# AndrewCullacino/handwritten-chinese-ocr-samples

Hardware: AMD Instinct MI355X
Metric: text-lines/sec (1x128x2000 synth) greedy decode (higher is better)
Workload: dtype f16 (f32 accumulate); 1 GPU; BASELINE configs[1]: 64 x 1x128x2000 uint8 lines, random-init hctr checkpoint (C=7358), forward + greedy CTC decode, labels to host; global_lines=64, lines_per_gpu=64, width=2000, classes=7358, checkpoint=random, parallelism=batch-shard x1

## Files before the change

handwritten-chinese-ocr-samples_amd/csrc/engine.cpp:

```cpp
#include "../../include/hctr_hip.h"
#include "kernels.h"

#include <algorithm>
#include <cfloat>
#include <cmath>
#include <cstdarg>
#include <cstdio>
#include <cstring>
#include <map>
#include <new>
#include <string>
#include <vector>

using namespace hctr;

namespace {

constexpr int kImgH = 128;
constexpr int kFeat = 2048;
constexpr double kBnEps = 1e-5;
constexpr int kStagePlanes[4] = {128, 256, 512, 512};
constexpr int kStageBlocks[4] = {2, 4, 5, 1};
constexpr int kStageH[5] = {128, 64, 32, 16, 8};
constexpr int64_t kDefaultMaxCols = 131072;

std::string g_create_error;

struct HostTensor {
    std::vector<float> data;
    std::vector<int64_t> shape;
    mutable bool used = false;
};

struct ConvW {
    half_t* w = nullptr;
    float* bias = nullptr;
    int cin = 0, cout = 0, coutPad = 0, taps = 0;
};

struct SeW {
    float* w1 = nullptr;
    float* w2 = nullptr;
    int c = 0;
};

struct BlockW {
    ConvW conv1, conv2, ds;
    SeW se;
    bool has_ds = false;
};

struct Workspace {
    int B = 0, W = 0, Wa = 0;
    void* img = nullptr;
    int32_t* widths = nullptr;
    half_t* s0 = nullptr;
    half_t* x[5] = {};
    half_t* p[5][3] = {};
    half_t* headin = nullptr;
    float* logits = nullptr;
    float* se_part = nullptr;
    float* se_scale = nullptr;
    float* se_border = nullptr;
    float* se_mean = nullptr;
    int32_t* se_counter = nullptr;
    int32_t* colidx = nullptr;
    float* amax_val = nullptr;
    int32_t* amax_idx = nullptr;
    int32_t* labels = nullptr;
    int32_t* lengths = nullptr;
    float* psum = nullptr;
    float* blank_logit = nullptr;
    float* row_thr = nullptr;
    int32_t* emit_cnt = nullptr;
    int32_t* emit_list = nullptr;
    double* esum = nullptr;
    int32_t* overflow = nullptr;
    int32_t* bm_idx = nullptr;
    float* bm_lp = nullptr;
    float* bm_bl = nullptr;
    float* bm_st = nullptr;
    int32_t* bm_cnt = nullptr;
    int32_t* tile_ctrs = nullptr;
    float* amax_val2 = nullptr;
    float* amax_abs = nullptr;
    float* col_margin = nullptr;
    float* col_abs = nullptr;
    float* line_guard = nullptr;
    int features = 0;
    bool split = false;
    bool aliased = false;
};

enum WsFeature { WS_S0 = 1, WS_LOGITS = 2, WS_BEAM = 4, WS_GUARD = 8 };

struct WeightSet {
    float* stem_w = nullptr;
    float* stem_b = nullptr;
    ConvW conv0_2;
    std::vector<BlockW> blocks[4];
    ConvW stage_conv[4];
    ConvW head;
    bool built = false;
};

struct ProfEntry {
    std::string name;
    hipEvent_t e0, e1;
};

}

struct hctr_ctx {
    int device = 0;
    int num_classes = 0;
    int cpad = 0;
    hipStream_t stream = nullptr;
    std::string err;
    std::map<std::string, HostTensor> host;
// ... 112 lines not shown
    for (void* p : pool) (void)hipFree(p);
    pool.clear();
}

struct PoolGuard {
    std::vector<void*>& pool;
    ~PoolGuard() { free_pool(pool); }
};

const HostTensor* find(hctr_ctx* c, const std::string& key) {
    auto it = c->host.find(key);
    return it == c->host.end() ? nullptr : &it->second;
}

int need(hctr_ctx* c, const std::string& key, std::vector<int64_t> shape, const HostTensor** out) {
    const HostTensor* t = find(c, key);
    if (!t) return fail(c, HCTR_ERR_KEY, "Missing key(s) in state_dict: \"%s\"", key.c_str());
    if (t->shape != shape) {
        std::string got, want;
        for (auto v : t->shape) got += std::to_string(v) + ",";
        for (auto v : shape) want += std::to_string(v) + ",";
        return fail(c, HCTR_ERR_SHAPE, "size mismatch for %s: checkpoint [%s] vs model [%s]", key.c_str(),
                    got.c_str(), want.c_str());
    }
    t->used = true;
    *out = t;
    return HCTR_OK;
}

inline int perm64(int s) {
    const int j = s >> 4, ra = s & 15;
    return (j >> 1) * 32 + (ra >> 2) * 8 + (j & 1) * 4 + (ra & 3);
}

int build_conv(hctr_ctx* c, const std::string& ck, const std::string& bk, int cin, int cout, int ks,
               bool has_bias, int pad_to, ConvW* out) {
    const HostTensor *w, *b = nullptr, *g, *beta, *mean, *var;
    TRY(need(c, ck + ".weight", {cout, cin, ks, ks}, &w));
    if (has_bias) TRY(need(c, ck + ".bias", {cout}, &b));
    TRY(need(c, bk + ".weight", {cout}, &g));
    TRY(need(c, bk + ".bias", {cout}, &beta));
    TRY(need(c, bk + ".running_mean", {cout}, &mean));
    TRY(need(c, bk + ".running_var", {cout}, &var));
    const int taps = ks * ks;
    const int coutPad = (cout + pad_to - 1) / pad_to * pad_to;
    const int cinp = c->chm() * cin;
    std::vector<half_t> hw((size_t)taps * coutPad * cinp, (half_t)0.f);
    std::vector<float> hb(coutPad, 0.f);
    double wmax = 0.0;
    for (int blk = 0; blk < coutPad / 64; ++blk)
        for (int s = 0; s < 64; ++s) {
            const int co = blk * 64 + perm64(s);
            if (co >= cout) continue;
            const double sc = (double)g->data[co] / std::sqrt((double)var->data[co] + kBnEps);
            for (int t = 0; t < taps; ++t)
                for (int ci = 0; ci < cin; ++ci) {
                    const double v = (double)w->data[((size_t)co * cin + ci) * taps + t] * sc;
                    wmax = std::max(wmax, std::fabs(v));
                    half_t* row = &hw[((size_t)t * coutPad + blk * 64 + s) * cinp];
                    const half_t hi = (half_t)(float)v;
                    row[ci] = hi;
                    if (c->split) {
                        row[cin + ci] = hi;
                        row[2 * cin + ci] = (c->x3_mask & 1) ? (half_t)(float)(v - (double)(float)hi) : (half_t)0.f;
                    }
                }
        }
    for (int co = 0; co < cout; ++co) {
        const double sc = (double)g->data[co] / std::sqrt((double)var->data[co] + kBnEps);
        const double bb = has_bias ? (double)b->data[co] : 0.0;
        hb[co] = (float)((bb - (double)mean->data[co]) * sc + (double)beta->data[co]);
    }
    if (!(wmax < 65000.0))
        return fail(c, HCTR_ERR_ARG, "%s: BatchNorm-folded weight magnitude %.3g does not fit fp16", ck.c_str(), wmax);
    out->cin = cinp; out->cout = cout; out->coutPad = coutPad; out->taps = taps;
    TRY(dev_alloc(c, c->wallocs, &out->w, hw.size(), false));
    TRY(dev_alloc(c, c->wallocs, &out->bias, hb.size(), false));
    HIP_TRY(c, hipMemcpyAsync(out->w, hw.data(), hw.size() * sizeof(half_t), hipMemcpyHostToDevice, c->stream));
    HIP_TRY(c, hipMemcpyAsync(out->bias, hb.data(), hb.size() * sizeof(float), hipMemcpyHostToDevice, c->stream));
    HIP_TRY(c, hipStreamSynchronize(c->stream));
    return HCTR_OK;
}

int build_se(hctr_ctx* c, const std::string& key, int ch, SeW* out) {
    const HostTensor *w1, *w2;
    TRY(need(c, key + ".fc.0.weight", {ch / 16, ch}, &w1));
    TRY(need(c, key + ".fc.2.weight", {ch, ch / 16}, &w2));
    out->c = ch;
    TRY(dev_alloc(c, c->wallocs, &out->w1, w1->data.size(), false));
    TRY(dev_alloc(c, c->wallocs, &out->w2, w2->data.size(), false));
    HIP_TRY(c, hipMemcpyAsync(out->w1, w1->data.data(), w1->data.size() * 4, hipMemcpyHostToDevice, c->stream));
    HIP_TRY(c, hipMemcpyAsync(out->w2, w2->data.data(), w2->data.size() * 4, hipMemcpyHostToDevice, c->stream));
    HIP_TRY(c, hipStreamSynchronize(c->stream));
    return HCTR_OK;
}

int build_stem(hctr_ctx* c, WeightSet& ws) {
    const HostTensor *w, *b, *g, *beta, *mean, *var;
    TRY(need(c, "cnn.conv0_1.weight", {64, 1, 3, 3}, &w));
    TRY(need(c, "cnn.conv0_1.bias", {64}, &b));
    TRY(need(c, "cnn.bn0_1.weight", {64}, &g));
    TRY(need(c, "cnn.bn0_1.bias", {64}, &beta));
    TRY(need(c, "cnn.bn0_1.running_mean", {64}, &mean));
    TRY(need(c, "cnn.bn0_1.running_var", {64}, &var));
    std::vector<float> hw(64 * 9), hb(64);
    for (int co = 0; co < 64; ++co) {
        const double sc = (double)g->data[co] / std::sqrt((double)var->data[co] + kBnEps);
        for (int t = 0; t < 9; ++t) hw[co * 9 + t] = (float)((double)w->data[co * 9 + t] * sc);
        hb[co] = (float)(((double)b->data[co] - (double)mean->data[co]) * sc + (double)beta->data[co]);
    }
    TRY(dev_alloc(c, c->wallocs, &ws.stem_w, hw.size(), false));
    TRY(dev_alloc(c, c->wallocs, &ws.stem_b, hb.size(), false));
    HIP_TRY(c, hipMemcpyAsync(ws.stem_w, hw.data(), hw.size() * 4, hipMemcpyHostToDevice, c->stream));
    HIP_TRY(c, hipMemcpyAsync(ws.stem_b, hb.data(), hb.size() * 4, hipMemcpyHostToDevice, c->stream));
    HIP_TRY(c, hipStreamSynchronize(c->stream));
    return HCTR_OK;
}

int build_head(hctr_ctx* c, WeightSet& ws) {
    const HostTensor *w, *b;
    const int C = c->num_classes;
    TRY(need(c, "linear.weight", {C, kFeat}, &w));
    TRY(need(c, "linear.bias", {C}, &b));
    const int cpad = c->cpad;
    const int kf = c->chm() * kFeat;
    std::vector<half_t> hw((size_t)cpad * kf, (half_t)0.f);
    std::vector<float> hb(cpad, 0.f);
    for (int blk = 0; blk < cpad / 64; ++blk)
        for (int s = 0; s < 64; ++s) {
            const int n = blk * 64 + perm64(s);
            if (n >= C) continue;
            half_t* dst = &hw[(size_t)(blk * 64 + s) * kf];
            const float* src = &w->data[(size_t)n * kFeat];
            for (int ch = 0; ch < 512; ++ch)
                for (int h = 0; h < 4; ++h) {
                    const float v = src[ch * 4 + h];
                    const half_t hi = (half_t)v;
                    if (!c->split) {
                        dst[h * 512 + ch] = hi;
                    } else {
                        half_t* r = dst + h * 1536;
                        r[ch] = hi;
                        r[512 + ch] = hi;
                        r[1024 + ch] = (c->x3_mask & 16) ? (half_t)(v - (float)hi) : (half_t)0.f;
                    }
                }
        }
    for (int n = 0; n < C; ++n) hb[n] = b->data[n];
    ws.head.cin = kf; ws.head.cout = C; ws.head.coutPad = cpad; ws.head.taps = 1;
    TRY(dev_alloc(c, c->wallocs, &ws.head.w, hw.size(), false));
    TRY(dev_alloc(c, c->wallocs, &ws.head.bias, hb.size(), false));
    HIP_TRY(c, hipMemcpyAsync(ws.head.w, hw.data(), hw.size() * sizeof(half_t), hipMemcpyHostToDevice, c->stream));
    HIP_TRY(c, hipMemcpyAsync(ws.head.bias, hb.data(), hb.size() * 4, hipMemcpyHostToDevice, c->stream));
    HIP_TRY(c, hipStreamSynchronize(c->stream));
    return HCTR_OK;
}

inline int64_t act_elems(int B, int H, int Wa, int C) { return (int64_t)B * (H + 2) * Wa * C; }

inline int head_parts_max(const hctr_ctx* c) { return c->cpad / 64; }
inline int head_parts(const hctr_ctx* c) {
    const int hbm = (c->big_tiles && c->cpad % 256 == 0) ? 256 : 128;
    return (c->cpad / hbm) * kLinearWN;
}

int ensure_workspace(hctr_ctx* c, int B, int W, int features = 0) {
// ... 146 lines not shown
        if (!on) return;
        ProfEntry pe{name, ev(), ev()};
        (void)hipEventRecord(pe.e0, c->stream);
        c->prof.push_back(pe);
    }
    void end() {
        if (!on) return;
        (void)hipEventRecord(c->prof.back().e1, c->stream);
    }
};

inline void prof_reset(hctr_ctx* c) {
    if (c->profiling) { c->prof.clear(); c->ev_used = 0; }
    c->h_widths.clear();
}

struct ActDesc {
    half_t* p;
    int H, C;
};

ConvTile pick_tile(const hctr_ctx* c, const ConvW& cw, int H) {
    if (cw.cout == 64) return TILE_64x256;
    if (c->halo_mode == 2 && cw.taps == 9 && cw.coutPad % 128 == 0 && H % 16 == 0) return TILE_HALO4;
    if (c->halo_mode == 2 && cw.taps == 9 && cw.coutPad % 128 == 0 && H % 8 == 0) return TILE_HALO4_8x32;
    if (c->big_tiles && cw.coutPad % 256 == 0 && H % 16 == 0) return TILE_256x256;
    return TILE_128x128;
}

int run_conv(hctr_ctx* c, Prof& pf, const char* name, const ConvW& cw, ActDesc in, half_t* out, int outH,
             bool relu, bool pool, float* se_part, bool to_head, const float* se_scale = nullptr,
             const half_t* resid = nullptr, const ConvW* ds = nullptr, const half_t* ds_in = nullptr,
             int stem_img_f32 = -1, bool stem_widths = false) {
    const Workspace& ws = c->ws;
    ConvArgs a{};
    a.x = in.p; a.w = cw.w; a.bias = cw.bias; a.y = out; a.se_part = se_part;
    a.se_scale = se_scale; a.resid = resid;
    a.split = c->split ? 1 : 0;
    a.drop_lo = (c->split && !(c->x3_mask & c->out_class)) ? 1 : 0;
    const int m = c->chm();
    a.H = in.H; a.W = ws.W; a.Cin = cw.cin; a.Cout = cw.cout; a.CoutPad = cw.coutPad;
    const ConvTile tile = pick_tile(c, cw, in.H);
    const int rows = conv_tile_rows(tile);
    if (in.H % rows != 0 || cw.cin % kBK != 0)
        return fail(c, HCTR_ERR_ARG, "conv %s: H=%d or Cin=%d not tileable", name, in.H, cw.cin);
    const int cols = conv_tile_cols(tile);
    a.tilesW = (ws.W + cols - 1) / cols;
    a.tilesH = in.H / rows;
    a.in_sb = (int64_t)(in.H + 2) * ws.Wa * cw.cin;
    a.in_sh = ws.Wa * cw.cin;
    if (a.in_sb * 2 >= ((int64_t)1 << 32) || (int64_t)(outH + 2) * ws.Wa * cw.cout * m * 2 >= ((int64_t)1 << 32))
        return fail(c, HCTR_ERR_ARG, "line width %d too large: one image's activation exceeds the kernels' 32-bit "
                    "in-image byte offsets (conv %s)", ws.W, name);
    if (to_head) {
        a.out_sb = (int64_t)ws.W * kFeat * m; a.out_sh = 512 * m; a.out_sw = kFeat * m; a.out_off = 0;
        a.out_wlimit = ws.W;
    } else {
        a.out_sb = (int64_t)(outH + 2) * ws.Wa * cw.cout * m;
        a.out_sh = ws.Wa * cw.cout * m; a.out_sw = cw.cout * m;
        a.out_off = (int64_t)(ws.Wa + 1) * cw.cout * m;
        a.out_wlimit = a.tilesW * cols;
    }
    a.relu = relu; a.pool = pool;
    if (ds) {
        if (tile != TILE_HALO4 || !se_scale || resid || ds->cin % kBK != 0 || ds->coutPad != cw.coutPad)
            return fail(c, HCTR_ERR_STATE, "conv %s: downsample fusion not applicable", name);
        a.ds_x = ds_in; a.ds_w = ds->w; a.ds_bias = ds->bias; a.ds_cin = ds->cin;
        a.ds_in_sh = ws.Wa * ds->cin;
        a.ds_in_sb = (int64_t)(in.H + 2) * ws.Wa * ds->cin;
    }
    a.mtiles = ws.B * a.tilesH * a.tilesW;
    a.ntiles = cw.coutPad / conv_tile_couts(tile);
    if (c->persist_dynamic && c->conv_seq < 64) a.tile_counter = ws.tile_ctrs + 8 * c->conv_seq++;
    if (c->stamp_buf && c->stamp_layer == name && (tile == TILE_HALO4 || tile == TILE_HALO4_8x32) &&
        (int64_t)a.mtiles * a.ntiles <= c->stamp_cap) {
        a.stamps = c->stamp_buf;
        c->stamp_n = (int64_t)a.mtiles * a.ntiles;
    }
    static const char* dbg_layer = getenv("HCTR_DBG_LAYER");
    if (dbg_layer && strcmp(dbg_layer, name) == 0)
        if (const char* e = getenv("HCTR_DBG")) a.dbg = atoi(e);
    pf.begin(name);
    if (stem_img_f32 >= 0) {
        if (tile != TILE_64x256 || cw.taps != 9 || cw.cin != 64 || cw.coutPad != 64 || c->split)
            return fail(c, HCTR_ERR_STATE, "conv %s: stem fusion not applicable", name);
        a.img = ws.img; a.img_f32 = stem_img_f32; a.img_widths = stem_widths ? ws.widths : nullptr;
        a.stem_w = c->wts().stem_w; a.stem_b = c->wts().stem_b;
        HIP_TRY(c, launch_stem_conv0_2(a, c->stream));
    } else {
        HIP_TRY(c, launch_conv(a, tile, cw.taps, false, c->stream));
    }
    pf.end();
    return HCTR_OK;
}

int run_block(hctr_ctx* c, Prof& pf, const std::string& name, const BlockW& bw, ActDesc in, half_t* t,
              half_t* o, half_t* r, int planes) {
    const Workspace& ws = c->ws;
    const int H = in.H;
    auto tiles_of = [&](const ConvW& cw) {
        const ConvTile t = pick_tile(c, cw, H);
        return (H / conv_tile_rows(t)) * ((ws.W + conv_tile_cols(t) - 1) / conv_tile_cols(t));
    };
    const float inv_hw = 1.0f / ((float)H * (float)ws.W);
    const half_t* res = in.p;
    const bool fuse_ds = bw.has_ds && c->fuse_ds && (c->fuse_se || c->split) && bw.ds.cin % kBK == 0 &&
                         pick_tile(c, bw.conv2, H) == TILE_HALO4;
    if (bw.has_ds && !fuse_ds) {
        c->out_class = 4;
        TRY(run_conv(c, pf, (name + ".downsample").c_str(), bw.ds, in, r, H, false, false, nullptr, false));
        res = r;
    }
    if (c->fuse_se || c->split) {
        const int tiles1 = tiles_of(bw.conv1);
        c->out_class = 2;
        TRY(run_conv(c, pf, (name + ".conv1").c_str(), bw.conv1, in, t, H, true, false, ws.se_part, false));
        c->out_class = 4;
        pf.begin((name + ".se_stats").c_str());
        HIP_TRY(c, launch_se_border(t, ws.B, H, ws.W, ws.Wa, planes, c->split, ws.se_part, tiles1, ws.se_border, c->stream));
        pf.end();
        pf.begin((name + ".se_scale").c_str());
        HIP_TRY(c, launch_se_premean(ws.se_border, t, bw.conv2.w, bw.conv2.bias, ws.B, H, ws.W, ws.Wa, planes,
                                     bw.conv2.coutPad, c->split, ws.se_mean, bw.se.w1, bw.se.w2, ws.se_scale,
                                     ws.se_counter, c->stream));
        pf.end();
        if (fuse_ds)
            TRY(run_conv(c, pf, (name + ".conv2+se+ds").c_str(), bw.conv2, ActDesc{t, H, planes}, o, H, true, false,
                         nullptr, false, ws.se_scale, nullptr, &bw.ds, in.p));
        else
            TRY(run_conv(c, pf, (name + ".conv2+se").c_str(), bw.conv2, ActDesc{t, H, planes}, o, H, true, false,
                         nullptr, false, ws.se_scale, res));
        return HCTR_OK;
    }
    c->out_class = 2;
    TRY(run_conv(c, pf, (name + ".conv1").c_str(), bw.conv1, in, t, H, true, false, nullptr, false));
    c->out_class = 4;
    TRY(run_conv(c, pf, (name + ".conv2").c_str(), bw.conv2, ActDesc{t, H, planes}, o, H, false, false,
                 ws.se_part, false));
    const int tiles = tiles_of(bw.conv2);
    pf.begin((name + ".se_fc").c_str());
    HIP_TRY(c, launch_se_fc(ws.se_part, tiles, bw.se.w1, bw.se.w2, ws.se_scale, ws.B, planes, inv_hw, c->stream));
    pf.end();
    pf.begin((name + ".se_apply").c_str());
    HIP_TRY(c, launch_se_apply(o, res, ws.se_scale, (int64_t)(H + 2) * ws.Wa * planes, ws.B, planes, c->stream));
    pf.end();
    return HCTR_OK;
}

enum HeadMode { HEAD_LOGITS = 0, HEAD_ARGMAX = 1, HEAD_BEAM = 2 };

int ws_need(const hctr_ctx* c, HeadMode mode, bool guarded = false) {
    int need = 0;
    if (mode == HEAD_LOGITS) need |= WS_LOGITS;
    if (mode == HEAD_BEAM) need |= WS_BEAM;
    if (!(c->fuse_stem && !c->split)) need |= WS_S0;
    if (guarded) need |= WS_GUARD;
    return need;
}

void head_args(hctr_ctx* c, ConvArgs* out, ConvTile* tile) {
    const Workspace& ws = c->ws;
    ConvArgs a{};
    a.x = ws.headin; a.w = c->wts().head.w; a.bias = c->wts().head.bias; a.y = ws.logits;
    a.Cin = c->wts().head.cin; a.Cout = c->num_classes; a.CoutPad = c->cpad;
    a.M = (int64_t)ws.B * ws.W; a.ldo = c->cpad;
    *tile = (c->big_tiles && c->cpad % 256 == 0) ? TILE_256x256 : TILE_128x128;
    const int hbm = *tile == TILE_256x256 ? 256 : 128;
    a.mtiles = (int)((a.M + hbm - 1) / hbm); a.ntiles = c->cpad / hbm;
// ... 386 lines not shown
            delete c;
            return fail(nullptr, HCTR_ERR_HIP, "hipStreamCreate: %s", hipGetErrorString(e));
        }
        if (const char* bt = getenv("HCTR_BIG_TILES")) c->big_tiles = atoi(bt) != 0;
        if (const char* hm = getenv("HCTR_HALO")) c->halo_mode = atoi(hm);
        if (const char* pr = getenv("HCTR_PRECISION")) {
            const std::string m(pr);
            c->mode = m == "f16x3" ? 1 : (m == "auto" ? 2 : 0);
            c->split = c->mode == 1;
        }
        if (const char* fs = getenv("HCTR_FUSE_SE")) c->fuse_se = atoi(fs) != 0;
        if (const char* fa = getenv("HCTR_FUSE_ARGMAX")) c->fuse_argmax = atoi(fa) != 0;
        if (const char* fd = getenv("HCTR_FUSE_DS")) c->fuse_ds = atoi(fd) != 0;
        if (const char* fb = getenv("HCTR_FUSE_BEAM")) c->fuse_beam = atoi(fb) != 0;
        if (const char* fs2 = getenv("HCTR_FUSE_STEM")) c->fuse_stem = atoi(fs2) != 0;
        if (const char* ps = getenv("HCTR_PERSIST")) c->persist_dynamic = atoi(ps) == 2;
        if (const char* xm = getenv("HCTR_X3_MASK")) c->x3_mask = atoi(xm) & 31;
        if (const char* wa = getenv("HCTR_WS_ALIAS")) c->ws_alias = atoi(wa) != 0 ? 1 : 0;
        if (const char* wd = getenv("HCTR_WS_DEDICATED_MAX_GB")) {
            const double g = atof(wd);
            if (g >= 0) c->ws_dedicated_max = (size_t)(g * 1073741824.0);
        }
        if (const char* mc = getenv("HCTR_MAX_COLS")) {
            const long long v = atoll(mc);
            if (v > 0) c->max_cols = v;
        }
        *out = c;
        return HCTR_OK;
    });
}

void hctr_destroy(hctr_ctx* c) {
    if (!c) return;
    (void)hipSetDevice(c->device);
    (void)hipStreamSynchronize(c->stream);
    if (c->arena) (void)hipFree(c->arena);
    if (c->pin) (void)hipHostFree(c->pin);
    free_pool(c->wallocs);
    free_pool(c->beam_allocs);
    if (c->ctc_buf) (void)hipFree(c->ctc_buf);
    if (c->stamp_buf) (void)hipFree(c->stamp_buf);
    for (hipEvent_t e : c->ev_pool) (void)hipEventDestroy(e);
    (void)hipStreamDestroy(c->stream);
    delete c;
}

const char* hctr_last_error(const hctr_ctx* c) { return c ? c->err.c_str() : g_create_error.c_str(); }

int hctr_load_tensor(hctr_ctx* c, const char* key, const void* host_ptr, const int64_t* shape, int ndim, int dtype) {
    return guard(c, [&]() -> int {
        if (!c) return HCTR_ERR_ARG;
        if (!key || (!host_ptr && ndim > 0) || ndim < 0 || ndim > 8) return fail(c, HCTR_ERR_ARG, "bad tensor arguments");
        if (c->finalized) return fail(c, HCTR_ERR_STATE, "weights already finalized");
        const std::string k(key);
        if (dtype == HCTR_I64) {
            if (k.size() < 19 || k.compare(k.size() - 19, 19, "num_batches_tracked") != 0)
                return fail(c, HCTR_ERR_KEY, "Unexpected key(s) in state_dict: \"%s\" (int64)", key);
            return HCTR_OK;
        }
        if (dtype != HCTR_F32) return fail(c, HCTR_ERR_ARG, "tensor %s: only float32 parameters are supported", key);
        HostTensor t;
        int64_t n = 1;
        for (int i = 0; i < ndim; ++i) {
            if (shape[i] < 0) return fail(c, HCTR_ERR_ARG, "negative dimension");
            t.shape.push_back(shape[i]);
            n *= shape[i];
        }
        t.data.assign((const float*)host_ptr, (const float*)host_ptr + n);
        c->host[k] = std::move(t);
        return HCTR_OK;
    });
}

int hctr_finalize_weights(hctr_ctx* c) {
    return guard(c, [&]() -> int {
        if (!c) return HCTR_ERR_ARG;
        if (c->finalized) return fail(c, HCTR_ERR_STATE, "weights already finalized");
        HIP_TRY(c, hipSetDevice(c->device));
        auto build_set = [&](bool split) -> int {
            c->split = split;
            WeightSet& ws = c->wset[split ? 1 : 0];
            TRY(build_stem(c, ws));
            TRY(build_conv(c, "cnn.conv0_2", "cnn.bn0_2", 64, 64, 3, true, 64, &ws.conv0_2));
            int inpl = 64;
            for (int s = 0; s < 4; ++s) {
                const int planes = kStagePlanes[s];
                ws.blocks[s].assign(kStageBlocks[s], BlockW());
                for (int i = 0; i < kStageBlocks[s]; ++i) {
                    BlockW& bw = ws.blocks[s][i];
                    const std::string p = "cnn.block" + std::to_string(s + 1) + "." + std::to_string(i);
                    if (i == 0 && inpl != planes) {
                        bw.has_ds = true;
                        TRY(build_conv(c, p + ".downsample.0", p + ".downsample.1", inpl, planes, 1, false, 128, &bw.ds));
                    }
                    TRY(build_conv(c, p + ".conv1", p + ".bn1", inpl, planes, 3, true, 128, &bw.conv1));
                    TRY(build_conv(c, p + ".conv2", p + ".bn2", planes, planes, 3, true, 128, &bw.conv2));
                    TRY(build_se(c, p + ".se", planes, &bw.se));
                    inpl = planes;
                }
                const std::string k = "cnn.conv" + std::to_string(s + 1);
                TRY(build_conv(c, k, "cnn.bn" + std::to_string(s + 1), planes, planes, 3, true, 128, &ws.stage_conv[s]));
            }
            TRY(build_head(c, ws));
            ws.built = true;
            return HCTR_OK;
        };
        int rc = HCTR_OK;
        if (c->mode != 1) rc = build_set(false);
        if (rc == HCTR_OK && c->mode != 0) rc = build_set(true);
        c->split = c->mode == 1;
        TRY(rc);
        for (auto& kv : c->host)
            if (!kv.second.used)
                return fail(c, HCTR_ERR_KEY, "Unexpected key(s) in state_dict: \"%s\"", kv.first.c_str());
        c->host.clear();
        c->finalized = true;
        return HCTR_OK;
    });
}

int hctr_set_precision(hctr_ctx* c, int mode) {
    return guard(c, [&]() -> int {
        if (!c) return HCTR_ERR_ARG;
        if (mode < 0 || mode > 2) return fail(c, HCTR_ERR_ARG, "precision mode must be 0 (f16), 1 (f16x3) or 2 (guarded: f16, "
                                                                 "uncertain lines again in f16x3)");
        if (c->finalized) {
            const bool need0 = mode != 1, need1 = mode != 0;
            if ((need0 && !c->wset[0].built) || (need1 && !c->wset[1].built))
                return fail(c, HCTR_ERR_STATE, "precision mode %d needs a weight set this context did not build: choose it "
                                               "(or mode 2) before hctr_finalize_weights", mode);
        }
        c->mode = mode;
        c->split = mode == 1;
        return HCTR_OK;
    });
}

int hctr_set_guard(hctr_ctx* c, double rel, double abs_tol) {
    return guard(c, [&]() -> int {
        if (!c) return HCTR_ERR_ARG;
        if (!(rel >= 0.0) || !(abs_tol >= 0.0)) return fail(c, HCTR_ERR_ARG, "guard tolerances must be >= 0");
        c->guard_rel = rel;
        c->guard_abs = abs_tol;
        return HCTR_OK;
    });
}

int hctr_last_guard(hctr_ctx* c, int64_t* lines, int64_t* flagged, uint8_t* flags, float* min_margin, float* scale,
                    int64_t cap) {
    return guard(c, [&]() -> int {
        if (!c) return HCTR_ERR_ARG;
        const int64_t n = (int64_t)c->g_flag.size();
        int64_t nf = 0;
        for (uint8_t f : c->g_flag) nf += f ? 1 : 0;
        if (lines) *lines = n;
        if (flagged) *flagged = nf;
        const int64_t m = n < cap ? n : (cap < 0 ? 0 : cap);
        if (flags && m) memcpy(flags, c->g_flag.data(), (size_t)m);
        if (min_margin && m) memcpy(min_margin, c->g_margin.data(), (size_t)m * 4);
        if (scale && m) memcpy(scale, c->g_scale.data(), (size_t)m * 4);
        return HCTR_OK;
    });
}

int hctr_workspace_stats(hctr_ctx* c, int64_t* arena_bytes, int64_t* arena_allocations, int64_t* recarves) {
    if (!c) return HCTR_ERR_ARG;
// ... 756 lines not shown
        for (int i = 0; i < n; ++i) {
            const int ch = channels[i];
            if (ch != 1 && ch != 3 && ch != -3) return fail(c, HCTR_ERR_ARG, "image %d: channels must be 1, 3 (BGR) or -3 (RGB)", i);
            if (heights[i] < 1 || widths[i] < 1) return fail(c, HCTR_ERR_SHAPE, "image %d: empty source", i);
            if (out_widths[i] < 1) return fail(c, HCTR_ERR_SHAPE, "image %d: destination width %d < 1", i, out_widths[i]);
            const int64_t bytes = (int64_t)heights[i] * widths[i] * (ch < 0 ? -ch : ch);
            if (offsets[i] < 0 || offsets[i] + bytes > packed_bytes)
                return fail(c, HCTR_ERR_ARG, "image %d: [%lld, +%lld) outside the packed buffer of %lld bytes", i,
                            (long long)offsets[i], (long long)bytes, (long long)packed_bytes);
            ResizeLine& L = lines[(size_t)i];
            L.src_off = offsets[i];
            L.sh = heights[i];
            L.sw = widths[i];
            L.ch = ch;
            L.dw = out_widths[i];
            L.inv_x = (double)L.dw / (double)L.sw;
            L.inv_y = (double)out_height / (double)L.sh;
            L.scale_x = 1.0 / L.inv_x;
            L.scale_y = 1.0 / L.inv_y;
            L.ix = (int)std::nearbyint(L.scale_x);
            L.iy = (int)std::nearbyint(L.scale_y);
            if (L.scale_x >= 1.0 && L.scale_y >= 1.0) {
                const bool fast = std::fabs(L.scale_x - L.ix) < DBL_EPSILON && std::fabs(L.scale_y - L.iy) < DBL_EPSILON;
                L.mode = fast ? 1 : 0;
            } else {
                L.mode = 2;
            }
        }
        HIP_TRY(c, hipSetDevice(c->device));
        std::vector<void*> tmp;
        PoolGuard tmp_guard{tmp};
        uint8_t *src = nullptr, *dst = nullptr;
        ResizeLine* dl = nullptr;
        int rc = dev_alloc(c, tmp, &src, (size_t)std::max<int64_t>(packed_bytes, 1), false);
        if (rc == HCTR_OK) rc = dev_alloc(c, tmp, &dl, (size_t)n, false);
        const size_t out_bytes = (size_t)n * out_height * out_W;
        if (rc == HCTR_OK && !out_on_device) rc = dev_alloc(c, tmp, &dst, out_bytes, false);
        if (rc == HCTR_OK) {
            uint8_t* target = out_on_device ? out : dst;
            hipError_t e = hipMemcpyAsync(src, packed_src, (size_t)packed_bytes, hipMemcpyHostToDevice, c->stream);
            if (e == hipSuccess)
                e = hipMemcpyAsync(dl, lines.data(), sizeof(ResizeLine) * (size_t)n, hipMemcpyHostToDevice, c->stream);
            if (e == hipSuccess) e = launch_resize_lines(src, dl, n, target, out_height, out_W, c->stream);
            if (e == hipSuccess && !out_on_device)
                e = hipMemcpyAsync(out, dst, out_bytes, hipMemcpyDeviceToHost, c->stream);
            if (e != hipSuccess) rc = fail(c, HCTR_ERR_HIP, "resize_lines: %s", hipGetErrorString(e));
        }
        hipError_t e = hipStreamSynchronize(c->stream);
        if (rc == HCTR_OK && e != hipSuccess) rc = fail(c, HCTR_ERR_HIP, "stream sync: %s", hipGetErrorString(e));
        free_pool(tmp);
        return rc;
    });
}

int64_t hctr_debug_stamps(hctr_ctx* c, const char* layer, uint64_t* out, int64_t cap_wgs) {
    return guard<int64_t>(c, [&]() -> int64_t {
        if (!c || cap_wgs < 0) return HCTR_ERR_ARG;
        if (hipSetDevice(c->device) != hipSuccess) return fail(c, HCTR_ERR_HIP, "hipSetDevice");
        if (layer) {
            if (c->stamp_buf) { (void)hipFree(c->stamp_buf); c->stamp_buf = nullptr; }
            c->stamp_layer = layer;
            c->stamp_cap = cap_wgs;
            c->stamp_n = 0;
            if (cap_wgs > 0 && hipMalloc((void**)&c->stamp_buf, (size_t)cap_wgs * 128) != hipSuccess)
                return fail(c, HCTR_ERR_NOMEM, "stamp buffer");
            return 0;
        }
        if (!out || !c->stamp_buf) return fail(c, HCTR_ERR_STATE, "stamping not armed");
        const int64_t n = std::min(c->stamp_n, cap_wgs);
        if (hipMemcpy(out, c->stamp_buf, (size_t)n * 128, hipMemcpyDeviceToHost) != hipSuccess)
            return fail(c, HCTR_ERR_HIP, "stamp copy");
        return n;
    });
}

int64_t hctr_debug_activation(hctr_ctx* c, const char* name, float* out, int64_t cap, int* Cout, int* Hout) {
    return guard<int64_t>(c, [&]() -> int64_t {
        if (!c || !name) return HCTR_ERR_ARG;
        const Workspace& ws = c->ws;
        if (ws.B == 0) return fail(c, HCTR_ERR_STATE, "no forward has run");
        const half_t* p = nullptr;
        int H = 0, C = 0;
        bool head = false;
        const std::string n(name);
        if (n == "conv0_1") {
            if (!ws.s0) return fail(c, HCTR_ERR_STATE, "conv0_1 is fused into conv0_2 (no buffer): use HCTR_FUSE_STEM=0");
            p = ws.s0; H = 128; C = 64;
        }
        else if (n == "stage0") { p = ws.x[1]; H = 64; C = 64; }
        else if (n == "stage1") { p = ws.x[2]; H = 32; C = 128; }
        else if (n == "stage2") { p = ws.x[3]; H = 16; C = 256; }
        else if (n == "stage3") { p = ws.x[4]; H = 8; C = 512; }
        else if (n == "stage4") { p = ws.headin; H = 4; C = 512; head = true; }
        else if (n.size() == 4 && n[0] == 'p' && n[2] == '.' && n[1] >= '1' && n[1] <= '4' && n[3] >= '0' && n[3] <= '2') {
            const int st = n[1] - '0', bi = n[3] - '0';
            p = ws.p[st][bi]; H = kStageH[st]; C = kStagePlanes[st - 1];
            if (!p) return fail(c, HCTR_ERR_ARG, "buffer %s not allocated", name);
        }
        else return fail(c, HCTR_ERR_ARG, "unknown activation '%s'", name);
        if (ws.aliased && !(n == "stage3" || n == "stage4" || (n.size() == 4 && n[0] == 'p' && n[1] == '4')))
            return fail(c, HCTR_ERR_STATE, "activation '%s' was overwritten by a later stage: the stages share their buffers "
                        "in this workspace layout (HCTR_WS_ALIAS=0 keeps every stage's own)", name);
        const int64_t total = (int64_t)ws.B * C * H * ws.W;
        if (Cout) *Cout = C;
        if (Hout) *Hout = H;
        if (!out || cap < total) return total;
        HIP_TRY(c, hipStreamSynchronize(c->stream));
        const int m = ws.split ? 3 : 1;
        const int64_t elems = head ? (int64_t)ws.B * ws.W * kFeat * m : act_elems(ws.B, H, ws.Wa, C * m);
        std::vector<half_t> host((size_t)elems);
        HIP_TRY(c, hipMemcpy(host.data(), p, (size_t)elems * sizeof(half_t), hipMemcpyDeviceToHost));
        for (int b = 0; b < ws.B; ++b)
            for (int ch = 0; ch < C; ++ch)
                for (int h = 0; h < H; ++h)
                    for (int w = 0; w < ws.W; ++w) {
                        const int64_t src = head ? (((int64_t)b * ws.W + w) * 4 + h) * (512 * m) + ch
                                                 : (((int64_t)b * (H + 2) + h + 1) * ws.Wa + w + 1) * (C * m) + ch;
                        float v = (float)host[(size_t)src];
                        if (m == 3) v += (float)host[(size_t)src + C];
                        out[(((int64_t)b * C + ch) * H + h) * ws.W + w] = v;
                    }
        return total;
    });
}

}
```

handwritten-chinese-ocr-samples_amd/csrc/kernels.hip:

```cpp
#include "kernels.h"

#include <cstdlib>

namespace hctr {

typedef _Float16 f16x8 __attribute__((ext_vector_type(8)));
typedef float f32x4 __attribute__((ext_vector_type(4)));
typedef float f32x2 __attribute__((ext_vector_type(2)));
typedef _Float16 f16x2 __attribute__((ext_vector_type(2)));
typedef uint32_t u32x4 __attribute__((ext_vector_type(4)));
typedef void __attribute__((address_space(3))) * lptr_t;

__device__ __forceinline__ void glds16_asm(const char* gsrc, char* lds_dst) {
    const uint32_t lds = (uint32_t)(uintptr_t)((lptr_t)lds_dst);
    uint32_t keep;
    asm volatile("s_mov_b32 %0, m0\n\ts_mov_b32 m0, %2\n\ts_nop 0\n\tglobal_load_lds_dwordx4 %1, off\n\ts_mov_b32 m0, %0"
                 : "=&s"(keep)
                 : "v"(gsrc), "s"(lds)
                 : "memory");
}

template <int CTRL>
__device__ __forceinline__ float dpp_f32(float v) {
    return __builtin_bit_cast(float, __builtin_amdgcn_update_dpp(0, __builtin_bit_cast(int, v), CTRL, 0xF, 0xF, true));
// ... 1547 lines not shown
    const int cg = threadIdx.x & 7;
    const int w = blockIdx.x * 32 + (threadIdx.x >> 3);
    const int h0 = blockIdx.y * kStemRows;
    const int b = blockIdx.z;
    if (w >= W) return;
    float wt[8][9], bs[8];
#pragma unroll
    for (int e = 0; e < 8; ++e) {
        bs[e] = bias[cg * 8 + e];
#pragma unroll
        for (int t = 0; t < 9; ++t) wt[e][t] = w9[(cg * 8 + e) * 9 + t];
    }
    const int wlim = widths ? widths[b] : W;
    auto pixel = [&](int hh, int ww) -> float {
        if (hh < 0 || hh >= 128 || ww < 0 || ww >= W) return 0.f;
        const int wsrc = ww < wlim ? ww : wlim - 1;
        const int64_t off = ((int64_t)b * 128 + hh) * W + wsrc;
        if (img_f32) return ((const float*)img)[off];
        float x = (float)((const uint8_t*)img)[off] / 255.0f;
        return (x - 0.5f) / 0.5f;
    };
    float win[3][3];
#pragma unroll
    for (int r = 0; r < 2; ++r)
#pragma unroll
        for (int d = 0; d < 3; ++d) win[r + 1][d] = pixel(h0 - 1 + r, w - 1 + d);
    const int cs = split ? 192 : 64;
    for (int r = 0; r < kStemRows; ++r) {
        const int h = h0 + r;
#pragma unroll
        for (int d = 0; d < 3; ++d) {
            win[0][d] = win[1][d];
            win[1][d] = win[2][d];
            win[2][d] = pixel(h + 1, w - 1 + d);
        }
        f16x8 o, ol;
#pragma unroll
        for (int e = 0; e < 8; ++e) {
            float sv = bs[e];
#pragma unroll
            for (int t = 0; t < 9; ++t) sv = fmaf(wt[e][t], win[t / 3][t % 3], sv);
            sv = fmaxf(sv, 0.f);
            o[e] = (half_t)sv;
            ol[e] = split == 2 ? (half_t)0.f : (half_t)(sv - (float)o[e]);
        }
        half_t* dst = y + (((int64_t)b * 130 + h + 1) * Wa + (w + 1)) * cs + cg * 8;
        *(f16x8*)dst = o;
        if (split) {
            *(f16x8*)(dst + 64) = ol;
            *(f16x8*)(dst + 128) = o;
        }
    }
}

__global__ __launch_bounds__(256) void zero_borders_kernel(half_t* __restrict__ p, int H, int W, int Wa, int C) {
    const int row = blockIdx.x, b = blockIdx.y;
    u32x4* r = (u32x4*)(p + ((int64_t)b * (H + 2) + row) * (int64_t)Wa * C);
    const int vpp = C >> 3;
    const u32x4 z = {0u, 0u, 0u, 0u};
    if (row == 0 || row == H + 1) {
        for (int i = threadIdx.x; i < Wa * vpp; i += 256) r[i] = z;
        return;
    }
    for (int i = threadIdx.x; i < vpp; i += 256) r[i] = z;
    const int first = (W + 1) * vpp, n = (Wa - W - 1) * vpp;
    for (int i = threadIdx.x; i < n; i += 256) r[first + i] = z;
}

hipError_t launch_zero_borders(half_t* p, int B, int H, int W, int Wa, int C, hipStream_t s) {
    if (B == 0) return hipSuccess;
    if (C % 8 != 0 || Wa < W + 2) return hipErrorInvalidValue;
    hipLaunchKernelGGL(zero_borders_kernel, dim3(H + 2, B), dim3(256), 0, s, p, H, W, Wa, C);
    return hipGetLastError();
}

hipError_t launch_stem(const void* img, int img_f32, const int32_t* widths_dev, const float* w9,
                       const float* bias, half_t* y, int B, int W, int Wa, int split, hipStream_t s) {
    if (B == 0) return hipSuccess;
    hipLaunchKernelGGL(stem_kernel, dim3((W + 31) / 32, 128 / kStemRows, B), dim3(256), 0, s, img, img_f32, widths_dev,
                       w9, bias, y, B, W, Wa, split);
    return hipGetLastError();
}

constexpr int kS2Halo = 32768;
constexpr int kS2Patch = 32768 + kHaloBytes;
constexpr int kS2Lds = kS2Patch + 20 * 20 * 4;

__global__ __launch_bounds__(256, 2) void stem_conv0_2_kernel(const ConvArgs a) {
    constexpr int JT = 4, S = kHaloCols;
    extern __shared__ __attribute__((aligned(16))) char smem[];
    const int tid = threadIdx.x;
    const int lane = tid & 63;
    const int wv = __builtin_amdgcn_readfirstlane(tid >> 6);
    const int total = a.mtiles;
    int lin;
    {
        const int id = blockIdx.x, xcd = id & 7, sl = id >> 3;
        const int qd = total >> 3, r = total & 7;
        lin = (xcd < r ? xcd * (qd + 1) : r * (qd + 1) + (xcd - r) * qd) + sl;
    }
    const int tw = lin % a.tilesW;
    const int t2 = lin / a.tilesW;
    const int th = t2 % a.tilesH;
    const int img = t2 / a.tilesH;
    const int W = a.W;

    auto stage_w = [&](int st, int buf) {
        const char* src = (const char*)a.w + (size_t)st * (2 * 64 * 64 * 2);
        char* dst = smem + buf * 16384 + (wv * 4) * 1024;
        const int npieces = st == 4 ? 8 : 16;
#pragma unroll
        for (int i = 0; i < 4; ++i) {
            const int piece = wv * 4 + i;
            if (piece < npieces) {
                const int g = piece * 64 + lane;
                const int row = g >> 3, cp = (g & 7) ^ (row & 7);
                glds16_asm(src + (uint32_t)row * 128u + cp * 16, dst + i * 1024);
            }
        }
    };
    stage_w(0, 0);
    stage_w(1, 1);

    float* patch = (float*)(smem + kS2Patch);
    {
        const int wlim = a.img_widths ? a.img_widths[img] : W;
        for (int e = tid; e < 400; e += 256) {
            const int py = e / 20, px = e - py * 20;
            const int hh = th * 16 - 2 + py, ww = tw * 16 - 2 + px;
            float v = 0.f;
            if (hh >= 0 && hh < 128 && ww >= 0 && ww < W) {
                const int wsrc = ww < wlim ? ww : wlim - 1;
                const int64_t off = ((int64_t)img * 128 + hh) * W + wsrc;
                if (a.img_f32) {
                    v = ((const float*)a.img)[off];
                } else {
                    const float x = (float)((const uint8_t*)a.img)[off] / 255.0f;
                    v = (x - 0.5f) / 0.5f;
                }
            }
            patch[e] = v;
        }
    }
    const int cg = tid & 7;
    float wt[8][9], bs[8];
    {
        const f32x4* wp = (const f32x4*)(a.stem_w + cg * 72);
        const f32x4* bp = (const f32x4*)(a.stem_b + cg * 8);
#pragma unroll
        for (int v = 0; v < 18; ++v) {
            const f32x4 w4 = wp[v];
#pragma unroll
            for (int i = 0; i < 4; ++i) wt[(v * 4 + i) / 9][(v * 4 + i) % 9] = w4[i];
        }
        const f32x4 b0 = bp[0], b1 = bp[1];
#pragma unroll
        for (int i = 0; i < 4; ++i) { bs[i] = b0[i]; bs[4 + i] = b1[i]; }
    }
    __syncthreads();
    for (int u = tid >> 3; u < kHaloRows * 18; u += 32) {
        const int hy = u / 18, hx = u - hy * 18;
        const int r = th * 16 - 1 + hy, col = tw * 16 - 1 + hx;
        f16x8 o;
        if (r >= 0 && r < 128 && col >= 0 && col < W) {
            float win[9];
#pragma unroll
            for (int t = 0; t < 9; ++t) win[t] = patch[(hy + t / 3) * 20 + hx + t % 3];
#pragma unroll
            for (int e = 0; e < 8; ++e) {
                float sv = bs[e];
#pragma unroll
                for (int t = 0; t < 9; ++t) sv = fmaf(wt[e][t], win[t], sv);
                o[e] = (half_t)fmaxf(sv, 0.f);
            }
        } else {
#pragma unroll
            for (int e = 0; e < 8; ++e) o[e] = (half_t)0.f;
        }
        const int hr = hy * S + hx;
        *(f16x8*)(smem + kS2Halo + hr * 128 + ((cg ^ (hr & 7)) << 4)) = o;
    }

    const int q = lane >> 4, c = lane & 15;
    const int aoff0 = c * 128 + (((0 + q) ^ (lane & 7)) << 4);
    const int aoff1 = c * 128 + (((4 + q) ^ (lane & 7)) << 4);
    const int wrow = wv * 4;
    f32x4 acc[JT][4];
#pragma unroll
    for (int j = 0; j < JT; ++j)
#pragma unroll
        for (int n = 0; n < 4; ++n) acc[j][n] = (f32x4){0.f, 0.f, 0.f, 0.f};
    for (int st = 0; st < 5; ++st) {
        asm volatile("s_waitcnt vmcnt(0)" ::: "memory");
        __syncthreads();
        if (st >= 1 && st + 1 < 5) stage_w(st + 1, (st + 1) & 1);
        const int ntap = st == 4 ? 1 : 2;
        for (int tt = 0; tt < ntap; ++tt) {
            const int tap = st * 2 + tt;
            const int tdy = tap / 3, dx = tap - tdy * 3 - 1;
            const int u = c + 1 + dx;
            const int v0 = u * 128 + (((q ^ (u & 7) ^ ((tdy & 1) << 2)) & 7) << 4);
            const char* hb = smem + kS2Halo + (wrow + tdy) * (S * 128);
            const char* be = hb + v0;
            const char* bo = hb + (v0 ^ 64);
            const char* wtile = smem + (st & 1) * 16384 + tt * 8192;
#pragma unroll
            for (int ks = 0; ks < 2; ++ks) {
                f16x8 af[JT], bf[4];
#pragma unroll
                for (int n = 0; n < 4; ++n) bf[n] = *(const f16x8*)((((n & 1) ^ ks) ? bo : be) + n * (S * 128));
#pragma unroll
                for (int j = 0; j < JT; ++j) af[j] = *(const f16x8*)(wtile + j * 2048 + (ks ? aoff1 : aoff0));
                __builtin_amdgcn_s_setprio(1);
#pragma unroll
                for (int j = 0; j < JT; ++j)
#pragma unroll
                    for (int n = 0; n < 4; ++n)
                        acc[j][n] = __builtin_amdgcn_mfma_f32_16x16x32_f16(af[j], bf[n], acc[j][n], 0, 0, 0);
                __builtin_amdgcn_s_setprio(0);
            }
        }
    }
    conv_epilogue<1, 4, JT, false, false>(a, acc, smem, tid, lane, 0, wv, 0, lin, img, th, tw, th * 16 + wrow, tw * 16);
}

hipError_t launch_stem_conv0_2(const ConvArgs& a, hipStream_t s) {
    if (a.mtiles == 0) return hipSuccess;
    static bool done[64] = {};
    hipError_t e0 = raise_lds_limit((const void*)stem_conv0_2_kernel, kS2Lds, done);
    if (e0 != hipSuccess) return e0;
    hipLaunchKernelGGL(stem_conv0_2_kernel, dim3(a.mtiles), dim3(256), kS2Lds, s, a);
    return hipGetLastError();
}

constexpr int kBorderSeg = 8;

__global__ __launch_bounds__(256) void se_border_kernel(const half_t* __restrict__ t, int H, int W, int Wa, int C,
                                                        int split, const float* __restrict__ tsum_part, int tiles,
                                                        float* __restrict__ out) {
    __shared__ float red[256 * 8];
    const int b = blockIdx.x, job = blockIdx.y;
    const int seg = blockIdx.z;
    if (job == 4) {
        const int per = (tiles + kBorderSeg - 1) / kBorderSeg;
        const int t0 = seg * per, t1 = t0 + per < tiles ? t0 + per : tiles;
        for (int ci = threadIdx.x; ci < C; ci += 256) {
            const float* p = tsum_part + (int64_t)b * tiles * C + ci;
            float s0 = 0.f, s1 = 0.f;
            int i = t0;
            for (; i + 1 < t1; i += 2) { s0 += p[(int64_t)i * C]; s1 += p[(int64_t)(i + 1) * C]; }
            if (i < t1) s0 += p[(int64_t)i * C];
            out[(((int64_t)b * 5 + 4) * kBorderSeg + seg) * C + ci] = s0 + s1;
        }
        return;
    }
    const int cv = C >> 3;
    const int v = threadIdx.x % cv, lanes = 256 / cv, p0 = threadIdx.x / cv;
    const int cs = split ? 3 * C : C;
    const half_t* img = t + (int64_t)b * (H + 2) * Wa * cs;
    const int count = job < 2 ? W : H;
    const int per = (count + kBorderSeg - 1) / kBorderSeg;
    const int pbeg = seg * per, pend = pbeg + per < count ? pbeg + per : count;
    float acc[8] = {0, 0, 0, 0, 0, 0, 0, 0};
    if (threadIdx.x < lanes * cv) {
        auto addr = [&](int p) {
            const int h = job == 0 ? 0 : (job == 1 ? H - 1 : p);
            const int w = job == 2 ? 0 : (job == 3 ? W - 1 : p);
            return img + ((int64_t)(h + 1) * Wa + (w + 1)) * cs + v * 8;
        };
        int p = pbeg + p0;
        for (; p + 3 * lanes < pend; p += 4 * lanes) {
            f16x8 x[4], xl[4];
#pragma unroll
            for (int u = 0; u < 4; ++u) {
                const half_t* px = addr(p + u * lanes);
                x[u] = *(const f16x8*)px;
                if (split) xl[u] = *(const f16x8*)(px + C);
            }
#pragma unroll
            for (int u = 0; u < 4; ++u) {
#pragma unroll
                for (int e = 0; e < 8; ++e) acc[e] += (float)x[u][e];
                if (split) {
#pragma unroll
                    for (int e = 0; e < 8; ++e) acc[e] += (float)xl[u][e];
                }
            }
        }
        for (; p < pend; p += lanes) {
            const half_t* px = addr(p);
            const f16x8 x = *(const f16x8*)px;
#pragma unroll
            for (int e = 0; e < 8; ++e) acc[e] += (float)x[e];
            if (split) {
                const f16x8 xl = *(const f16x8*)(px + C);
#pragma unroll
                for (int e = 0; e < 8; ++e) acc[e] += (float)xl[e];
            }
        }
    }
#pragma unroll
    for (int e = 0; e < 8; ++e) red[threadIdx.x * 8 + e] = acc[e];
    __syncthreads();
    if (threadIdx.x < cv) {
        float s[8] = {0, 0, 0, 0, 0, 0, 0, 0};
        for (int l = 0; l < lanes; ++l)
#pragma unroll
            for (int e = 0; e < 8; ++e) s[e] += red[(l * cv + threadIdx.x) * 8 + e];
#pragma unroll
        for (int e = 0; e < 8; ++e)
            out[(((int64_t)b * 5 + job) * kBorderSeg + seg) * C + threadIdx.x * 8 + e] = s[e];
    }
}

// ... 1376 lines not shown
```

Measured before the change: 502.1 lines/s.

## Load stem conv0_2 weights as prepacked MFMA fragments from global, drop LDS staging

The fused stem conv0_2 kernel no longer stages its weights through 32 KB of LDS. Weights are repacked once at load time into per-lane MFMA A-fragment order and read straight from global/L2 into registers, double-buffered per tap. This removes the LDS weight buffers and their barriers, so LDS use shrinks enough to allow three workgroups per CU instead of two. The cost is more register pressure from the 2x8 fragment buffers and repeated global weight reads per workgroup. A '+border' padded activation debug view is also added.

```diff
diff --git a/handwritten-chinese-ocr-samples_amd/csrc/engine.cpp b/handwritten-chinese-ocr-samples_amd/csrc/engine.cpp
--- a/handwritten-chinese-ocr-samples_amd/csrc/engine.cpp
+++ b/handwritten-chinese-ocr-samples_amd/csrc/engine.cpp
@@ -35,6 +35,7 @@
 struct ConvW {
     half_t* w = nullptr;
     float* bias = nullptr;
+    half_t* wfrag = nullptr;
     int cin = 0, cout = 0, coutPad = 0, taps = 0;
 };
 
@@ -313,6 +314,25 @@
     return HCTR_OK;
 }
 
+int pack_stem_frags(hctr_ctx* c, ConvW* cw) {
+    if (cw->taps != 9 || cw->cin != 64 || cw->coutPad != 64) return fail(c, HCTR_ERR_STATE, "pack_stem_frags: not conv0_2");
+    std::vector<half_t> hw((size_t)9 * 64 * 64), pk(hw.size());
+    HIP_TRY(c, hipMemcpyAsync(hw.data(), cw->w, hw.size() * sizeof(half_t), hipMemcpyDeviceToHost, c->stream));
+    HIP_TRY(c, hipStreamSynchronize(c->stream));
+    for (int tap = 0; tap < 9; ++tap)
+        for (int ks = 0; ks < 2; ++ks)
+            for (int j = 0; j < 4; ++j)
+                for (int lane = 0; lane < 64; ++lane) {
+                    const int q = lane >> 4, cc = lane & 15;
+                    const half_t* src = &hw[((size_t)tap * 64 + j * 16 + cc) * 64 + (ks * 4 + q) * 8];
+                    std::copy(src, src + 8, &pk[((((size_t)tap * 2 + ks) * 4 + j) * 64 + lane) * 8]);
+                }
+    TRY(dev_alloc(c, c->wallocs, &cw->wfrag, pk.size(), false));
+    HIP_TRY(c, hipMemcpyAsync(cw->wfrag, pk.data(), pk.size() * sizeof(half_t), hipMemcpyHostToDevice, c->stream));
+    HIP_TRY(c, hipStreamSynchronize(c->stream));
+    return HCTR_OK;
+}
+
 int build_se(hctr_ctx* c, const std::string& key, int ch, SeW* out) {
     const HostTensor *w1, *w2;
     TRY(need(c, key + ".fc.0.weight", {ch / 16, ch}, &w1));
@@ -625,8 +645,9 @@
         if (const char* e = getenv("HCTR_DBG")) a.dbg = atoi(e);
     pf.begin(name);
     if (stem_img_f32 >= 0) {
-        if (tile != TILE_64x256 || cw.taps != 9 || cw.cin != 64 || cw.coutPad != 64 || c->split)
+        if (tile != TILE_64x256 || cw.taps != 9 || cw.cin != 64 || cw.coutPad != 64 || c->split || !cw.wfrag)
             return fail(c, HCTR_ERR_STATE, "conv %s: stem fusion not applicable", name);
+        a.w = cw.wfrag;
         a.img = ws.img; a.img_f32 = stem_img_f32; a.img_widths = stem_widths ? ws.widths : nullptr;
         a.stem_w = c->wts().stem_w; a.stem_b = c->wts().stem_b;
         HIP_TRY(c, launch_stem_conv0_2(a, c->stream));
@@ -1179,6 +1200,7 @@
             WeightSet& ws = c->wset[split ? 1 : 0];
             TRY(build_stem(c, ws));
             TRY(build_conv(c, "cnn.conv0_2", "cnn.bn0_2", 64, 64, 3, true, 64, &ws.conv0_2));
+            if (!split) TRY(pack_stem_frags(c, &ws.conv0_2));
             int inpl = 64;
             for (int s = 0; s < 4; ++s) {
                 const int planes = kStagePlanes[s];
@@ -2101,7 +2123,9 @@
         const half_t* p = nullptr;
         int H = 0, C = 0;
         bool head = false;
-        const std::string n(name);
+        std::string n(name);
+        const bool padded = n.size() > 7 && n.compare(n.size() - 7, 7, "+border") == 0;
+        if (padded) n.resize(n.size() - 7);
         if (n == "conv0_1") {
             if (!ws.s0) return fail(c, HCTR_ERR_STATE, "conv0_1 is fused into conv0_2 (no buffer): use HCTR_FUSE_STEM=0");
             p = ws.s0; H = 128; C = 64;
@@ -2120,15 +2144,25 @@
         if (ws.aliased && !(n == "stage3" || n == "stage4" || (n.size() == 4 && n[0] == 'p' && n[1] == '4')))
             return fail(c, HCTR_ERR_STATE, "activation '%s' was overwritten by a later stage: the stages share their buffers "
                         "in this workspace layout (HCTR_WS_ALIAS=0 keeps every stage's own)", name);
-        const int64_t total = (int64_t)ws.B * C * H * ws.W;
+        if (padded && (head || ws.split)) return fail(c, HCTR_ERR_ARG, "'%s': no padded view of this buffer", name);
+        const int64_t total = padded ? (int64_t)ws.B * C * (H + 2) * ws.Wa : (int64_t)ws.B * C * H * ws.W;
         if (Cout) *Cout = C;
-        if (Hout) *Hout = H;
+        if (Hout) *Hout = padded ? H + 2 : H;
         if (!out || cap < total) return total;
         HIP_TRY(c, hipStreamSynchronize(c->stream));
         const int m = ws.split ? 3 : 1;
         const int64_t elems = head ? (int64_t)ws.B * ws.W * kFeat * m : act_elems(ws.B, H, ws.Wa, C * m);
         std::vector<half_t> host((size_t)elems);
         HIP_TRY(c, hipMemcpy(host.data(), p, (size_t)elems * sizeof(half_t), hipMemcpyDeviceToHost));
+        if (padded) {
+            for (int b = 0; b < ws.B; ++b)
+                for (int ch = 0; ch < C; ++ch)
+                    for (int h = 0; h < H + 2; ++h)
+                        for (int w = 0; w < ws.Wa; ++w)
+                            out[(((int64_t)b * C + ch) * (H + 2) + h) * ws.Wa + w] =
+                                (float)host[(size_t)((((int64_t)b * (H + 2) + h) * ws.Wa + w) * C + ch)];
+            return total;
+        }
         for (int b = 0; b < ws.B; ++b)
             for (int ch = 0; ch < C; ++ch)
                 for (int h = 0; h < H; ++h)
diff --git a/handwritten-chinese-ocr-samples_amd/csrc/kernels.hip b/handwritten-chinese-ocr-samples_amd/csrc/kernels.hip
--- a/handwritten-chinese-ocr-samples_amd/csrc/kernels.hip
+++ b/handwritten-chinese-ocr-samples_amd/csrc/kernels.hip
@@ -1653,13 +1653,14 @@
     return hipGetLastError();
 }
 
-constexpr int kS2Halo = 32768;
-constexpr int kS2Patch = 32768 + kHaloBytes;
+constexpr int kS2Halo = 0;
+constexpr int kS2Patch = kHaloBytes;
 constexpr int kS2Lds = kS2Patch + 20 * 20 * 4;
-
-__global__ __launch_bounds__(256, 2) void stem_conv0_2_kernel(const ConvArgs a) {
+static_assert(3 * kS2Lds <= 160 * 1024, "three workgroups per CU");
+
+__global__ __launch_bounds__(256, 3) void stem_conv0_2_kernel(const ConvArgs a) {
     constexpr int JT = 4, S = kHaloCols;
-    extern __shared__ __attribute__((aligned(16))) char smem[];
+    __shared__ __attribute__((aligned(16))) char smem[kS2Lds];
     const int tid = threadIdx.x;
     const int lane = tid & 63;
     const int wv = __builtin_amdgcn_readfirstlane(tid >> 6);
@@ -1676,22 +1677,11 @@
     const int img = t2 / a.tilesH;
     const int W = a.W;
 
-    auto stage_w = [&](int st, int buf) {
-        const char* src = (const char*)a.w + (size_t)st * (2 * 64 * 64 * 2);
-        char* dst = smem + buf * 16384 + (wv * 4) * 1024;
-        const int npieces = st == 4 ? 8 : 16;
-#pragma unroll
-        for (int i = 0; i < 4; ++i) {
-            const int piece = wv * 4 + i;
-            if (piece < npieces) {
-                const int g = piece * 64 + lane;
-                const int row = g >> 3, cp = (g & 7) ^ (row & 7);
-                glds16_asm(src + (uint32_t)row * 128u + cp * 16, dst + i * 1024);
-            }
-        }
+    const u32x4* wfrag = (const u32x4*)a.w + lane;
+    auto load_w = [&](int tap, u32x4 (&wf)[8]) {
+#pragma unroll
+        for (int f = 0; f < 8; ++f) wf[f] = wfrag[(tap * 8 + f) * 64];
     };
-    stage_w(0, 0);
-    stage_w(1, 1);
 
     float* patch = (float*)(smem + kS2Patch);
     {
@@ -1752,55 +1742,47 @@
         *(f16x8*)(smem + kS2Halo + hr * 128 + ((cg ^ (hr & 7)) << 4)) = o;
     }
 
+    u32x4 wf[2][8];
+    load_w(0, wf[0]);
+    __syncthreads();
     const int q = lane >> 4, c = lane & 15;
-    const int aoff0 = c * 128 + (((0 + q) ^ (lane & 7)) << 4);
-    const int aoff1 = c * 128 + (((4 + q) ^ (lane & 7)) << 4);
     const int wrow = wv * 4;
     f32x4 acc[JT][4];
 #pragma unroll
     for (int j = 0; j < JT; ++j)
 #pragma unroll
         for (int n = 0; n < 4; ++n) acc[j][n] = (f32x4){0.f, 0.f, 0.f, 0.f};
-    for (int st = 0; st < 5; ++st) {
-        asm volatile("s_waitcnt vmcnt(0)" ::: "memory");
-        __syncthreads();
-        if (st >= 1 && st + 1 < 5) stage_w(st + 1, (st + 1) & 1);
-        const int ntap = st == 4 ? 1 : 2;
-        for (int tt = 0; tt < ntap; ++tt) {
-            const int tap = st * 2 + tt;
-            const int tdy = tap / 3, dx = tap - tdy * 3 - 1;
-            const int u = c + 1 + dx;
-            const int v0 = u * 128 + (((q ^ (u & 7) ^ ((tdy & 1) << 2)) & 7) << 4);
-            const char* hb = smem + kS2Halo + (wrow + tdy) * (S * 128);
-            const char* be = hb + v0;
-            const char* bo = hb + (v0 ^ 64);
-            const char* wtile = smem + (st & 1) * 16384 + tt * 8192;
-#pragma unroll
-            for (int ks = 0; ks < 2; ++ks) {
-                f16x8 af[JT], bf[4];
-#pragma unroll
-                for (int n = 0; n < 4; ++n) bf[n] = *(const f16x8*)((((n & 1) ^ ks) ? bo : be) + n * (S * 128));
-#pragma unroll
-                for (int j = 0; j < JT; ++j) af[j] = *(const f16x8*)(wtile + j * 2048 + (ks ? aoff1 : aoff0));
-                __builtin_amdgcn_s_setprio(1);
-#pragma unroll
-                for (int j = 0; j < JT; ++j)
-#pragma unroll
-                    for (int n = 0; n < 4; ++n)
-                        acc[j][n] = __builtin_amdgcn_mfma_f32_16x16x32_f16(af[j], bf[n], acc[j][n], 0, 0, 0);
-                __builtin_amdgcn_s_setprio(0);
-            }
-        }
+#pragma unroll
+    for (int tap = 0; tap < 9; ++tap) {
+        if (tap + 1 < 9) load_w(tap + 1, wf[(tap + 1) & 1]);
+        const int tdy = tap / 3, dx = tap - tdy * 3 - 1;
+        const int u = c + 1 + dx;
+        const int v0 = u * 128 + (((q ^ (u & 7) ^ ((tdy & 1) << 2)) & 7) << 4);
+        const char* hb = smem + kS2Halo + (wrow + tdy) * (S * 128);
+        const char* be = hb + v0;
+        const char* bo = hb + (v0 ^ 64);
+#pragma unroll
+        for (int ks = 0; ks < 2; ++ks) {
+            f16x8 bf[4];
+#pragma unroll
+            for (int n = 0; n < 4; ++n) bf[n] = *(const f16x8*)((((n & 1) ^ ks) ? bo : be) + n * (S * 128));
+            __builtin_amdgcn_s_setprio(1);
+#pragma unroll
+            for (int j = 0; j < JT; ++j)
+#pragma unroll
+                for (int n = 0; n < 4; ++n)
+                    acc[j][n] = __builtin_amdgcn_mfma_f32_16x16x32_f16(__builtin_bit_cast(f16x8, wf[tap & 1][ks * 4 + j]),
+                                                                       bf[n], acc[j][n], 0, 0, 0);
+            __builtin_amdgcn_s_setprio(0);
+        }
+        __builtin_amdgcn_sched_barrier(0);
     }
     conv_epilogue<1, 4, JT, false, false>(a, acc, smem, tid, lane, 0, wv, 0, lin, img, th, tw, th * 16 + wrow, tw * 16);
 }
 
 hipError_t launch_stem_conv0_2(const ConvArgs& a, hipStream_t s) {
     if (a.mtiles == 0) return hipSuccess;
-    static bool done[64] = {};
-    hipError_t e0 = raise_lds_limit((const void*)stem_conv0_2_kernel, kS2Lds, done);
-    if (e0 != hipSuccess) return e0;
-    hipLaunchKernelGGL(stem_conv0_2_kernel, dim3(a.mtiles), dim3(256), kS2Lds, s, a);
+    hipLaunchKernelGGL(stem_conv0_2_kernel, dim3(a.mtiles), dim3(256), 0, s, a);
     return hipGetLastError();
 }
 
```

Measured after the change: 504.4 lines/s (median of 6 runs). Within noise of the previous version (+0.5%).
